# SeanNobel/speech-decoding

Hardware: AMD Instinct MI355X
Metric: train segments/sec (Gwilliams2022 208ch x 360, top-10 retrieval acc alongside) (higher is better)
Workload: dtype bf16; 1 GPU; Gwilliams2022-shaped MEG: 208 ch x 360 samples, 27 subjects, F=1024, batch 256/GPU, fwd+CLIP loss+top-k+bwd+Adam (BASELINE configs[1]); global_batch=256, seq_len=360, parallelism=dp1

## Files before the change

### include/sd_amd.h

```cpp
#ifndef SD_AMD_H
#define SD_AMD_H
#include <stddef.h>
#include <stdint.h>

#ifdef __cplusplus
extern "C" {
#endif

#define SDA_ABI_VERSION 4
#define SDA_ROW_PAD 16
#define SDA_CH_ALIGN 64

enum { SDA_F32 = 0, SDA_BF16 = 1, SDA_F16 = 2 };

enum { SDA_EPI_GELU = 1,
       SDA_EPI_GLU_BWD = 4,
       SDA_EPI_GLU = 2,
       SDA_CONV_SINGLE_TILE = 4096,
       SDA_CONV_PAIR_TILES = 8192,
       SDA_CONV_ONE_PER_CU = 32768,
       SDA_CONV_FLAT_TILES = 16384,
       SDA_CONV_FLAT_STAGGER = 1024,
       SDA_CONV_WIDE_TILES = 524288,
       SDA_CONV_WAVE_PRIO = 1048576,
// ... 95 lines not shown
                                    float* dgamma, float* dbeta, float* coef, void* dx, int B, int T, int Cp, int dtype,
                                    void* stream);
int sda_bn_gelu_backward_apply_dg(const void* dy, const void* x, const float* mean, const float* rstd,
                               const float* gamma, const float* beta, int C, const float* dgamma,
                               const float* dbeta, double count, float* coef , void* dx,
                               int B, int T, int Cp, int dtype, void* stream);

int sda_reduce_scratch_floats(int Cp);

int sda_zero_pad_rows(void* buf, int B, int T, int Cp, int dtype, void* stream);
int sda_fill_zero(void* p, long nbytes, void* stream);
int sda_gather_samples(const void* table, const long* idx, void* dst, int B, long sample_bytes, void* stream);
int sda_gather_windows(const void* table, long table_rows, const int32_t* starts, int M, const long* idx, void* dst, int B, int T,
                       long row_bytes, void* stream);
int sda_scalar_mul(const float* a, const float* b, float* out, int n, void* stream);

int sda_glu_forward(const void* x, void* y, int B, int T, int Ch, int dtype, void* stream);
int sda_glu_backward(const void* x, const void* dy, void* dx, int B, int T, int Ch, int dtype, void* stream);
int sda_gelu_backward(const void* u, const void* dz, void* du, int B, int T, int Cp, int dtype, void* stream);
int sda_reduce_scratch_rows(int B, int T);
int sda_glu_backward_colsum(const void* x, const void* dy, void* dx, float* colsum, float* scratch, int B, int T,
                            int Ch, int dtype, void* stream);
int sda_gelu_backward_colsum(const void* u, const void* dz, void* du, float* colsum, float* scratch, int B, int T,
                             int Cp, int dtype, void* stream);
int sda_glu_backward_colsum_og(const void* out, const void* gate, const void* dy, void* dx, float* colsum, float* scratch,
                               int B, int T, int Ch, int dtype, void* stream);
int sda_colsum(const void* x, float* out, float* scratch , int B, int T,
               int Cp, int dtype, void* stream);

enum { SDA_WGRAD_FLAT_ROWS = 1   };
typedef struct sda_wgrad_args {
  const void* dy;
  const void* x;
  float* g;
  void* out_e;
  const void* sub;
  const float* rscale;
  const float* out_scale;
  const int32_t* perm;
  const int32_t* seg_start;
  int nseg, B, T, Cout_p, Cin_p, KS, dil;
  long dy_pitch, x_pitch, out_pitch;
  long row0, sample_rows;
  long rows_limit;
  long dy_zero_row;
  int co_valid;
  int dtype;
  const float* acc_scale;
  int flags;
} sda_wgrad_args;
int sda_wgrad_gemm(const sda_wgrad_args* a, void* stream);
int sda_wgrad_tile_m(int Cout_p);
int sda_reduce_slabs(const float* src, float* dst, int nslabs, long n, void* stream);
int sda_sim_gemm_ksplit(int M, int N, long K, int dtype);
int sda_sim_gemm(const void* X, const void* W, float* partial, int M, int N, int Np, long K, long pitch, int ksplit, int dtype,
                 void* stream);
int sda_sim_gemm_windows(const void* X, long x_pitch, const void* table, const int32_t* starts, int base_row, long row_elems,
                         float* partial, int M, int N, int Np, long K, int ksplit, int dtype, void* stream);
long sda_sim_gemm_windows_span(long row_elems);
int sda_window_sumsq(const float* row_sq, const int32_t* starts, float* out, int M, int T, void* stream);

int sda_sa_weights_forward(const float* z, const float* cos_t, const float* sin_t, const float* mask,
                           float* W, void* Wp, float* scratch , int D1, int K2,
                           int C, int D1p, int Cp, int dtype, void* stream);
int sda_sa_scratch_floats(int D1, int K2, int C);
int sda_sa_softmax_pack(const float* a, int a_pitch, const float* mask, float* W, void* Wp, int D1, int C, int D1p,
                        int Cp, int dtype, void* stream);
int sda_sa_softmax_backward(const float* dWd, int dwd_pitch, const float* W, const float* mask, float* da,
                            int da_pitch, int D1, int C, void* stream);
int sda_sa_weights_backward(const float* dWd, const float* W, const float* mask, const float* cosT,
                            const float* sinT, float* dz, int D1, int K2, int C, int Cp, void* stream);

int sda_clip_logits_stats(const float* S, long s_pitch, const float* ysq, const float* zsq, const float* temp,
                          float* logits, float* row_max, float* row_sum, float* col_lse, float* diag , float* row_lse ,
                          int Bm, int Bn, int col0, void* stream);
int sda_clip_grad(const float* logits, const float* row_lse, const float* col_lse, const float* ysq,
                  const float* zsq, const float* temp, float inv_norm, int col0, void* G, long g_pitch,
                  float* rscale, float* cscale, float* colpart, float* scalars, int Bm, int Bn, int dtype, void* stream);
int sda_clip_grad_y(const float* logits, const float* row_lse, const float* col_lse, const float* zsq,
                    const float* zsq_all, int nz, int col0, void* Gy, long gy_pitch, int seg, int seg_pitch,
                    float* part, int Bm, int Bn, int dtype, void* stream);
int sda_clip_grad_y_finish(const float* part, int nparts, int Bg, const float* ysq, const float* zsq_all, int nz,
                           const float* temp, float inv_norm, int row0, int nrows, float* rscale_y, float* cscale_y,
                           void* stream);
int sda_clip_dz_supported(int Bm, int Bn, long row_elems, int dtype);
int sda_clip_dz(const void* G, long g_pitch, const void* Y, const void* Z, void* out, const float* cscale, const float* rscale,
                const float* out_scale, int Bm, int Bn, long row_elems, int dtype, void* stream);
int sda_clip_ranks(const float* logits, const float* diag, int32_t* cnt, int Bm, int Bn, int col0, void* stream);
long sda_retrieval_scores_floats(int n, int M, int chunk_cols);
int sda_retrieval_select(const float* S, const float* qsq, const float* csq, const int64_t* labels, int64_t* indices,
                         float* scores, int32_t* ranks, int n, int M, int k, int chunk_cols, void* stream);
int sda_retrieval_class_reduce(const float* S, const float* qsq, const float* csq, const int32_t* order, const int32_t* offsets,
                               float* out, float* row_lse, long out_pitch, int n, int M, int C, int chunk_cols, float scale,
                               int mode, void* stream);
int sda_retrieval_pool_rows(const float* V, long v_pitch, const int32_t* rows, const int32_t* group_offsets, float* out,
                            long out_pitch, int N, int G, int C, void* stream);
int sda_clip_merge_rows(const float* all, int world, int Bg, float* lse, float* diag, void* stream);
int sda_device_count(void);
int sda_stream_create_cumask(const uint32_t* mask, int nwords, void** stream);
int sda_stream_create_priority(int priority, void** stream);
int sda_stream_destroy(void* stream);
int sda_set_cu_limit(int cus);

typedef struct sda_pgemm_args {
  const float* A;
  const float* B;
// ... 95 lines not shown
```

### speech_decoding_amd/blocks.py

```python
from __future__ import annotations

from dataclasses import dataclass, field
from typing import Dict, Optional

import numpy as np
import torch

from . import lib as L
from . import layers
from . import ops

FWD_FLAGS = L.CONV_PAIR_TILES
BWD_FLAGS = L.CONV_WAVE_PRIO


def rows_in(X: torch.Tensor, Cc: int, dtype):
    if X.dtype not in ops.COMPUTE_DTYPES:
        raise L.SdaError(f"input of dtype {X.dtype}: the modules take float32, bfloat16 or float16")
    return ops.rows_of(X, Cc, dtype, ops.new_rows_uninit)


def grad_rows(dY: torch.Tensor, Cc: int, dtype) -> torch.Tensor:
    return ops.rows_of(dY, Cc, dtype, ops.new_rows_uninit)[0]

# ... 49 lines not shown
    dX = ops.input_grad(dY, c.Wp, None, c.B, Cc, c.T, c.x_dtype) if want_x else None
    dz = None
    if want_z:
        dz = layers.sa_z_grad(dY, c.Xt, c.B, c.T, *_segments(c.B, dY, c.Xt), c.W, c.mask, *sa.transposed_tables(), sa.z.shape[1],
                              sa.gemm_tables()[1])
    return dX, dz


def spatial_attention_forward(sa, X: torch.Tensor, mask, need_grad: bool):
    B, Cc, T = X.shape
    Xt, _ = rows_in(X, Cc, sa.compute_dtype)
    y, W, Wp = sa_forward(sa, Xt, B, T, mask, sa.compute_dtype)
    return y, (SACtx(B, T, Xt, W, Wp, mask, X.dtype) if need_grad else None)


@dataclass
class SBCtx:
    sa: SACtx
    h_sa: torch.Tensor
    h_c: torch.Tensor
    widx: torch.Tensor
    subj: Optional[tuple] = None
    params: list = field(default_factory=list)
    versions: list = field(default_factory=list)


def _sb_plans(sb):
    D1p = L.pad_channels(sb.D1)

    def build(f, b):
        layers.add_subject_block_packs(f, b, sb.conv.weight, sb.conv.bias, sb.subject_layer.weight, D1p)
        return f, b
    return _plans(sb, sb.conv.weight.device, build)


def _sb_sources(sb) -> Dict[str, torch.Tensor]:
    return {"sb_w": sb.conv.weight.detach(), "sb_b": sb.conv.bias.detach(), "subj_w": sb.subject_layer.weight.detach()}


def subject_block_forward(sb, X: torch.Tensor, sidx: np.ndarray, mask, need_grad: bool, want_subj_grad: bool):
    B, Cc, T = X.shape
    dt, dev, D1, S = sb.compute_dtype, X.device, sb.D1, sb.num_subjects
    D1p = L.pad_channels(D1)
    widx = ops.UPLOADER.upload("blocks.widx", sidx.astype(np.int32), dev)
    Xt, _ = rows_in(X, Cc, dt)
    h_sa, W, Wp = sa_forward(sb.spatial_attention, Xt, B, T, mask, dt)
    pk = _sb_plans(sb)[0].run(_sb_sources(sb))
    h_c = ops.conv_gemm(h_sa, pk["sb_w"], _new(B, T, D1p, dt, dev), B=B, T=T, KS=1, dil=0, bias=pk["sb_b"], alg_dims=(D1, D1))
    y = ops.conv_gemm(h_c, pk["subj_w"], _new(B, T, D1p, dt, dev), B=B, T=T, KS=1, dil=0, widx=widx, alg_dims=(D1, D1))
    if not need_grad:
        return y, None
    c = SBCtx(SACtx(B, T, Xt, W, Wp, mask, X.dtype), h_sa, h_c, widx)
    if want_subj_grad:
        plan = layers.subject_plan(sidx, S, *layers.subject_tiles_blocks(D1p))
        c.subj = (ops.UPLOADER.upload("blocks.subj_perm", plan.perm, dev), ops.UPLOADER.upload("blocks.subj_seg", plan.seg_start, dev),
                  plan.r)
    return y, c


def subject_block_backward(sb, c: SBCtx, dY: torch.Tensor, want: Dict[str, bool]) -> Dict[str, torch.Tensor]:
    _check_versions(c)
    B, T, dt, dev = c.sa.B, c.sa.T, sb.compute_dtype, dY.device
    D1, S = sb.D1, sb.num_subjects
    D1p = L.pad_channels(D1)
    g: Dict[str, torch.Tensor] = {}
    if want["subj_w"]:
        g["subj_w"] = layers.subject_wgrad(dY, c.h_c, B, T, *c.subj, S, D1)
    if not (want["sb_w"] or want["sb_b"] or want["z"] or want["X"]):
        return g
    pkT = _sb_plans(sb)[1].run(_sb_sources(sb))
    dh_c = ops.conv_gemm(dY, pkT["subj_w"], _new(B, T, D1p, dt, dev), B=B, T=T, KS=1, dil=0, widx=c.widx, alg_dims=(D1, D1),
                         flags=BWD_FLAGS)
    if want["sb_w"]:
        g["sb_w"] = _wgrad(dh_c, c.h_sa, B, T, 1, 0, D1, D1)
    if want["sb_b"]:
        g["sb_b"] = ops.colsum(dh_c, B, T, ops.reduce_scratch(D1p, dev))[:D1]
    if want["z"] or want["X"]:
        dh_sa = ops.conv_gemm(dh_c, pkT["sb_w"], _new(B, T, D1p, dt, dev), B=B, T=T, KS=1, dil=0, alg_dims=(D1, D1),
                              flags=BWD_FLAGS)
        g["X"], g["z"] = sa_backward(sb.spatial_attention, c.sa, dh_sa, want["X"], want["z"])
    return g


CB_PARAMS = ("c0w", "c0b", "bn0w", "bn0b", "c1w", "c1b", "bn1w", "bn1b", "c2w", "c2b")


def cb_params(cb):
    return [cb.conv0.weight, cb.conv0.bias, cb.batchnorm0.weight, cb.batchnorm0.bias, cb.conv1.weight, cb.conv1.bias,
            cb.batchnorm1.weight, cb.batchnorm1.bias, cb.conv2.weight, cb.conv2.bias]


@dataclass
class CBCtx:
    B: int
    T: int
    x: torch.Tensor
    x_rows: bool
    x_dtype: torch.dtype
    h: list
    a: list
    bn: list
    c2: torch.Tensor
    params: list = field(default_factory=list)
    versions: list = field(default_factory=list)


def _cb_plans(cb):
    def build(f, b):
        layers.add_conv_block_packs(f, b, "", [(c.weight, c.bias) for c in (cb.conv0, cb.conv1, cb.conv2)], cb.D2,
                                    L.pad_channels(cb.in_channels))
        return f, b
    return _plans(cb, cb.conv0.weight.device, build)


def _cb_sources(cb) -> Dict[str, torch.Tensor]:
    return {n: p.detach() for n, p in zip(CB_PARAMS, cb_params(cb)) if not n.startswith("bn")}


def conv_block_forward(cb, X: torch.Tensor, need_grad: bool):
    B, Cc, T = X.shape
# ... 81 lines not shown
```

### speech_decoding_amd/csrc/param_ops.hip

```cpp
#include <math.h>

#include "sd_common.h"

namespace sda {

__device__ inline int glu_unmap(int cop, int Cout, int half, int half_p, int tile = 0) {
  if (half == 0) return cop < Cout ? cop : -1;
  if (tile > 0) {
    const int j = cop / (2 * tile), w = cop - j * 2 * tile;
    const int r = j * tile + (w < tile ? w : w - tile);
    if (w < tile) return r < half ? r : -1;
    return r < Cout - half ? half + r : -1;
  }
  if (cop < half_p) return cop < half ? cop : -1;
  const int r = cop - half_p;
  return r < Cout - half ? half + r : -1;
}
__device__ inline int glu_map(int co, int half, int half_p) { return (half == 0 || co < half) ? co : half_p + co - half; }

__device__ inline float packed_weight_value(const float* __restrict__ w, size_t i, int Cout, int Cin, int KS, int Cout_p,
                                            int Cin_p, int mode, int half, int half_p, int tile) {
  int co, ci, tap;
  size_t q = i;
  if (mode == 0) {
// ... 49 lines not shown

__device__ inline void slab_add(float& s, float v) { s += v; }
__device__ inline void slab_add(float4& s, const float4& v) { s.x += v.x; s.y += v.y; s.z += v.z; s.w += v.w; }

template <typename V>
__device__ inline V ordered_slab_sum(const float* __restrict__ slabs, int nslabs, size_t slab, size_t src) {
  V sum = {};
  int k = 0;
  for (; k + 8 <= nslabs; k += 8) {
    V v[8];
#pragma unroll
    for (int j = 0; j < 8; ++j) v[j] = *reinterpret_cast<const V*>(slabs + (size_t)(k + j) * slab + src);
#pragma unroll
    for (int j = 0; j < 8; ++j) slab_add(sum, v[j]);
  }
  for (; k < nslabs; ++k) slab_add(sum, *reinterpret_cast<const V*>(slabs + (size_t)k * slab + src));
  return sum;
}

__global__ void reduce_unpack_wgrad_kernel(const float* __restrict__ slabs, int nslabs, float* __restrict__ dst, int Cout,
                                           int Cin, int KS, int Cout_p, int Cin_p, int half, int half_p) {
  const size_t total = (size_t)Cout * Cin * KS;
  const size_t slab = (size_t)KS * Cout_p * Cin_p;
  for (size_t i = (size_t)blockIdx.x * blockDim.x + threadIdx.x; i < total; i += (size_t)gridDim.x * blockDim.x) {
    size_t q = i;
    const int ci = q % Cin; q /= Cin;
    const int co = q % Cout; q /= Cout;
    const int tap = (int)q;
    const size_t src = ((size_t)tap * Cout_p + glu_map(co, half, half_p)) * Cin_p + ci;
    dst[((size_t)co * Cin + ci) * KS + tap] = ordered_slab_sum<float>(slabs, nslabs, slab, src);
  }
}

__global__ __launch_bounds__(256) void reduce_unpack_wgrad_vec_kernel(const float* __restrict__ slabs, int nslabs, float* __restrict__ dst,
                                                                      int Cout, int Cin, int KS, int Cout_p, int Cin_p, int half, int half_p) {
  const int cin4 = Cin >> 2;
  const size_t total = (size_t)Cout * cin4 * KS;
  const size_t slab = (size_t)KS * Cout_p * Cin_p;
  for (size_t i = (size_t)blockIdx.x * blockDim.x + threadIdx.x; i < total; i += (size_t)gridDim.x * blockDim.x) {
    size_t q = i;
    const int c4 = q % cin4; q /= cin4;
    const int co = q % Cout; q /= Cout;
    const int tap = (int)q;
    const size_t src = ((size_t)tap * Cout_p + glu_map(co, half, half_p)) * Cin_p + 4 * c4;
    const float4 sum = ordered_slab_sum<float4>(slabs, nslabs, slab, src);
    float* o = dst + ((size_t)co * Cin + 4 * c4) * KS + tap;
    o[0] = sum.x; o[KS] = sum.y; o[2 * KS] = sum.z; o[3 * KS] = sum.w;
  }
}

__global__ void reduce_slabs_kernel(const float* __restrict__ src, float* __restrict__ dst, int nslabs, long n) {
  for (long i = (long)blockIdx.x * blockDim.x + threadIdx.x; i < n; i += (long)gridDim.x * blockDim.x)
    dst[i] = ordered_slab_sum<float>(src, nslabs, (size_t)n, (size_t)i);
}

__global__ void pack_vector_kernel(const float* __restrict__ v, float* __restrict__ dst, int C, int Cp, int half, int half_p) {
  const int i = blockIdx.x * blockDim.x + threadIdx.x;
  if (i >= Cp) return;
  const int c = glu_unmap(i, C, half, half_p);
  dst[i] = c >= 0 ? v[c] : 0.f;
}
__global__ void unpack_vector_kernel(const float* __restrict__ g, float* __restrict__ dst, int C, int half, int half_p) {
  const int i = blockIdx.x * blockDim.x + threadIdx.x;
  if (i < C) dst[i] = g[glu_map(i, half, half_p)];
}

static inline int ew_grid(size_t total) {
  size_t g = (total + 255) / 256;
  return (int)(g < 1 ? 1 : (g > 4096 ? 4096 : g));
}

}

using namespace sda;

extern "C" int sda_pack_conv_weight(const float* w, void* dst, int nW, int Cout, int Cin, int KS, int Cout_p,
                                    int Cin_p, int mode, int glu_half, int glu_half_p, int dtype, void* stream) {
  if (!w || !dst || nW < 1 || Cout > Cout_p || Cin > Cin_p || (mode != 0 && mode != 1)) { set_error("pack_conv_weight: bad arguments"); return -1; }
  if (glu_half && (glu_half_p < glu_half || glu_half_p + (Cout - glu_half) > Cout_p)) { set_error("pack_conv_weight: bad GLU split"); return -1; }
  hipStream_t st = (hipStream_t)stream;
  const size_t total = (size_t)nW * KS * Cout_p * Cin_p;
  SDA_DISPATCH(dtype, hipLaunchKernelGGL(pack_conv_weight_kernel<E>, dim3(ew_grid(total)), dim3(256), 0, st, w,
                                         (E*)dst, nW, Cout, Cin, KS, Cout_p, Cin_p, mode, glu_half, glu_half_p));
  return check_launch("pack_conv_weight");
}

extern "C" int sda_unpack_conv_wgrad(const float* g, float* dst, int nW, int Cout, int Cin, int KS, int Cout_p,
                                     int Cin_p, int glu_half, int glu_half_p, void* stream) {
  if (!g || !dst) { set_error("unpack_conv_wgrad: null"); return -1; }
  const size_t total = (size_t)nW * Cout * Cin * KS;
  hipLaunchKernelGGL(unpack_conv_wgrad_kernel, dim3(ew_grid(total)), dim3(256), 0, (hipStream_t)stream, g, dst, nW,
                     Cout, Cin, KS, Cout_p, Cin_p, glu_half, glu_half_p);
  return check_launch("unpack_conv_wgrad");
}

template <bool COEF>
__device__ __forceinline__ void adam_multi_body(const sda_adam_desc& d, float lr, float beta1, float beta2, float eps, float bc1,
                                                float bc2_sqrt, float coef) {
  const float step_size = lr / bc1;
  for (long i = ((long)blockIdx.x * 256 + threadIdx.x) * 4; i < d.n; i += (long)gridDim.x * 1024) {
    if (i + 4 <= d.n && d.aligned) {
      float4 p = *reinterpret_cast<float4*>(d.param + i);
      float4 g = *reinterpret_cast<const float4*>(d.grad + i);
      if (COEF) { g.x = __fmul_rn(g.x, coef); g.y = __fmul_rn(g.y, coef); g.z = __fmul_rn(g.z, coef); g.w = __fmul_rn(g.w, coef); }
      float4 m = *reinterpret_cast<float4*>(d.exp_avg + i), v = *reinterpret_cast<float4*>(d.exp_avg_sq + i);
#define SDA_ADAM(f)                                                     \
// ... 33 lines not shown
}

extern "C" int sda_adam_multi(const sda_adam_desc* descs_dev, int n, long max_n, float lr, float beta1, float beta2, float eps,
                              long step, void* stream) {
  if (!descs_dev || n < 1 || max_n < 1 || step < 1) { set_error("adam_multi: bad arguments"); return -1; }
  const double bc1 = 1.0 - pow((double)beta1, (double)step);
  const double bc2 = 1.0 - pow((double)beta2, (double)step);
  long gx = (max_n + 1023) / 1024;
  if (gx > 256) gx = 256;
  hipLaunchKernelGGL(adam_multi_kernel, dim3((unsigned)gx, (unsigned)n), dim3(256), 0, (hipStream_t)stream, descs_dev, lr, beta1,
                     beta2, eps, (float)bc1, (float)sqrt(bc2));
  return check_launch("adam_multi");
}

extern "C" int sda_adam_multi_guarded(const sda_adam_desc* descs_dev, int n, long max_n, float lr, float beta1, float beta2,
                                      float eps, const double* state, void* stream) {
  if (!descs_dev || !state || n < 1 || max_n < 1) { set_error("adam_multi_guarded: bad arguments (null pointer, n or max_n < 1)"); return -1; }
  long gx = (max_n + 1023) / 1024;
  if (gx > 256) gx = 256;
  hipLaunchKernelGGL(adam_multi_guarded_kernel, dim3((unsigned)gx, (unsigned)n), dim3(256), 0, (hipStream_t)stream, descs_dev, lr,
                     beta1, beta2, eps, state);
  return check_launch("adam_multi_guarded");
}

extern "C" int sda_pack_multi(const sda_pack_desc* descs_dev, int n, long max_total, int dtype, void* stream) {
  if (!descs_dev || n < 1 || max_total < 1) { set_error("pack_multi: bad arguments"); return -1; }
  hipStream_t st = (hipStream_t)stream;
  long gx = (max_total + 1023) / 1024;
  if (gx > 512) gx = 512;
  SDA_DISPATCH(dtype, hipLaunchKernelGGL(pack_multi_kernel<E>, dim3((unsigned)gx, (unsigned)n), dim3(256), 0, st, descs_dev));
  return check_launch("pack_multi");
}

extern "C" int sda_reduce_unpack_wgrad(const float* slabs, int nslabs, float* dst, int Cout, int Cin, int KS, int Cout_p,
                                       int Cin_p, int glu_half, int glu_half_p, void* stream) {
  if (!slabs || !dst || nslabs < 1) { set_error("reduce_unpack_wgrad: bad arguments"); return -1; }
  const size_t total = (size_t)Cout * Cin * KS;
  if (Cin % 4 == 0 && Cin_p % 4 == 0 && (reinterpret_cast<uintptr_t>(slabs) & 15) == 0) {
    hipLaunchKernelGGL(reduce_unpack_wgrad_vec_kernel, dim3(ew_grid(total / 4)), dim3(256), 0, (hipStream_t)stream, slabs, nslabs, dst,
                       Cout, Cin, KS, Cout_p, Cin_p, glu_half, glu_half_p);
    return check_launch("reduce_unpack_wgrad");
  }
  hipLaunchKernelGGL(reduce_unpack_wgrad_kernel, dim3(ew_grid(total)), dim3(256), 0, (hipStream_t)stream, slabs, nslabs, dst,
                     Cout, Cin, KS, Cout_p, Cin_p, glu_half, glu_half_p);
  return check_launch("reduce_unpack_wgrad");
}

extern "C" int sda_reduce_slabs(const float* src, float* dst, int nslabs, long n, void* stream) {
  if (!src || !dst || nslabs < 1 || n < 1) { set_error("reduce_slabs: bad arguments"); return -1; }
  hipLaunchKernelGGL(reduce_slabs_kernel, dim3(ew_grid((size_t)n)), dim3(256), 0, (hipStream_t)stream, src, dst, nslabs, n);
  return check_launch("reduce_slabs");
}

extern "C" int sda_pack_vector(const float* v, float* dst, int C, int Cp, int glu_half, int glu_half_p, void* stream) {
  if (!v || !dst || C > Cp) { set_error("pack_vector: bad arguments"); return -1; }
  hipLaunchKernelGGL(pack_vector_kernel, dim3((Cp + 255) / 256), dim3(256), 0, (hipStream_t)stream, v, dst, C, Cp,
                     glu_half, glu_half_p);
  return check_launch("pack_vector");
}

extern "C" int sda_unpack_vector(const float* g, float* dst, int C, int Cp, int glu_half, int glu_half_p, void* stream) {
  if (!g || !dst || C > Cp) { set_error("unpack_vector: bad arguments"); return -1; }
  hipLaunchKernelGGL(unpack_vector_kernel, dim3((C + 255) / 256), dim3(256), 0, (hipStream_t)stream, g, dst, C,
                     glu_half, glu_half_p);
  return check_launch("unpack_vector");
}
```

### speech_decoding_amd/engine.py

```python
from __future__ import annotations

from dataclasses import dataclass, field
from typing import Dict, List, Optional

import ast
import os

import numpy as np
import torch

from . import lib as L
from . import layers
from . import ops
from .clip import ClipBlockStats, ClipCtx, clip_backward, clip_backward_y, clip_block_finish, clip_block_stats, clip_forward


@dataclass
class EncoderDims:
    C: int
    S: int
    D1: int
    D2: int
    F: int
    K: int

    @property
    def Cp(self): return L.pad_channels(self.C)
    @property
    def D1p(self): return L.pad_channels(self.D1)
    @property
    def D2p(self): return L.pad_channels(self.D2)
    @property
    def F1(self): return 2 * self.D2
    @property
    def F1p(self): return L.pad_channels(2 * self.D2)
    @property
    def Fp(self): return L.pad_channels(self.F)


@dataclass
class EncoderCtx:
    B: int
    T: int
    gen: int
    training: bool
    bufs: Dict[str, torch.Tensor] = field(default_factory=dict)
    packed: Dict[str, torch.Tensor] = field(default_factory=dict)
    bn: Dict[str, tuple] = field(default_factory=dict)
    mask: Optional[torch.Tensor] = None
    widx: Optional[torch.Tensor] = None
    subj_perm: Optional[torch.Tensor] = None
    subj_seg: Optional[torch.Tensor] = None
    subj_slices: int = 1
    W_sa: Optional[torch.Tensor] = None
    packed_T: Dict[str, torch.Tensor] = field(default_factory=dict)
    packed_T_ready: Optional[torch.cuda.Event] = None
    glu_fused: bool = False
    composed: Optional[tuple] = None
    param_grads: bool = True
    x_dtype: Optional[torch.dtype] = None
    W_x: Optional[torch.Tensor] = None


@dataclass
class _Forward:
    eng: "EncoderEngine"
    P: Dict[str, torch.Tensor]
    ctx: EncoderCtx
    dev: torch.device
    main: torch.cuda.Stream
    need_grad: bool
    need_dx: bool
    eps: float
    momentum: float
    k3_flags: int
    count: float
    packed_ready: Optional[torch.cuda.Event] = None
    flip: Dict[int, int] = field(default_factory=dict)

    def rows(self, name, Cp):
        B, T = self.ctx.B, self.ctx.T
        if not self.need_grad:
            name = f"pp{self.flip.setdefault(Cp, 0) % 3}"
            self.flip[Cp] += 1
        return self.eng._rows(name, B, T, Cp, self.dev, "train" if self.need_grad else "eval")


class _Backward:
    __slots__ = ("eng", "P", "ctx", "B", "T", "dev", "pg", "main", "side", "grads", "pending", "scratch", "overlap", "world")

    def __init__(self, eng: "EncoderEngine", P, ctx: EncoderCtx, dev, main):
        d = eng.d
        self.eng, self.P, self.ctx, self.B, self.T, self.dev, self.main = eng, P, ctx, ctx.B, ctx.T, dev, main
        self.grads: Dict[str, torch.Tensor] = {}
        self.pg = ctx.param_grads
        self.scratch = ops.reduce_scratch(max(d.Fp, 2 * d.D2p, d.F1p), dev)
        self.pending = []
        self.overlap = eng.group is not None and eng.overlap_grad_allreduce
        self.side = eng._side_stream(dev) if eng.wgrad_side_stream else None
        self.world = eng.world

    def flush(self, names):
        if not self.overlap or not self.pg:
            return
        import torch.distributed as dist
        from .distributed import side_group
# ... 184 lines not shown
            layers.add_conv_block_packs(f, b, f"b{k}.", [(P[f"b{k}.c{j}w"], P[f"b{k}.c{j}b"]) for j in range(3)], d.D2,
                                        d.D1p if k == 0 else d.D2p, glu_tile)
        f.add_weight("f1w", P["f1w"], d.F1p, d.D2p)
        f.add_vector("f1b", P["f1b"], d.F1p)
        f.add_weight("f2w", P["f2w"], d.Fp, d.F1p)
        f.add_vector("f2b", P["f2b"], d.Fp)
        b.add_weight("f1w", P["f1w"], d.F1p, d.D2p, mode=1)
        b.add_weight("f2w", P["f2w"], d.Fp, d.F1p, mode=1)
        self._fwd_plan, self._bwd_plan, self._plan_key = f, b, key
        return f, b

    def forward(self, P: Dict[str, torch.Tensor], X: torch.Tensor, subject_idxs, *, training: bool,
                mask: Optional[torch.Tensor], need_grad: bool, momentum: float = 0.1, eps: float = 1e-5,
                need_dx: bool = False, param_grads: bool = True) -> EncoderCtx:
        B, Cc, T = X.shape
        assert Cc == self.d.C, f"expected {self.d.C} channels, got {Cc}"
        dev = X.device
        if need_grad:
            self._gen += 1
        self._touch_shape("train" if need_grad else "eval", B, T)
        ctx = EncoderCtx(B=B, T=T, gen=self._gen, training=training)
        ctx.glu_fused = self.glu_fused
        if need_dx and not need_grad:
            raise L.SdaError("EncoderEngine.forward: need_dx needs need_grad")
        ctx.param_grads = bool(param_grads or not need_dx)
        ctx.x_dtype = X.dtype if need_dx else None
        ctx.mask = mask
        k3_flags = L.CONV_PAIR_TILES
        if self.flat_forward:
            k3_flags |= L.CONV_FLAT_TILES | L.CONV_FLAT_STAGGER
        f = _Forward(self, P, ctx, dev, torch.cuda.current_stream(dev), need_grad, need_dx, eps, momentum, k3_flags,
                     count=float(B) * T * self.world)

        self._fwd_subjects(f, subject_idxs)
        Xt = ctx.bufs["Xt"] = self._fwd_pack(f, X)
        x = self._fwd_subject_block(f, Xt)
        for k in range(5):
            x = self._fwd_conv_block(f, k, x)
        Zt = self._fwd_projections(f, x)
        if not need_grad:
            ctx.bufs = {"Z": Zt}
            ctx.packed = {}
        return ctx

    def _fwd_subjects(self, f: _Forward, subject_idxs):
        d, ctx = self.d, f.ctx
        B = ctx.B
        sidx = layers.subject_indices(subject_idxs, B, d.S)
        up = ops.UPLOADER.upload
        ctx.widx = up(("widx", "train" if f.need_grad else "eval"), sidx.astype(np.int32), f.dev)
        if not (f.need_grad and ctx.param_grads):
            return
        tiles = layers.subject_tiles_composed(d.D2p, d.Cp) if self.composed else layers.subject_tiles_three_conv(d.D1p)
        plan = layers.subject_plan(sidx, d.S, *tiles)
        ctx.subj_perm = up("subj_perm", plan.perm, f.dev)
        ctx.subj_seg = up("subj_seg", plan.seg_start, f.dev)
        ctx.subj_slices = plan.r

    def _fwd_pack(self, f: _Forward, X):
        d, ctx, P = self.d, f.ctx, f.P
        fwd_plan, bwd_plan = self._plans(P, f.dev)
        side = self._side_stream(f.dev) if self.pack_on_side_stream else None
        Xt = f.rows("Xt", d.Cp)
        if side is not None:
            ev = torch.cuda.Event()
            ev.record(f.main)
            side.wait_event(ev)
        with torch.cuda.stream(side):
            ctx.packed.update(fwd_plan.run(P))
            ops.pack_rows(X, Xt, ones_channel=d.C if self.composed else None)
            if side is not None:
                X.record_stream(side)
                f.packed_ready = torch.cuda.Event()
                f.packed_ready.record(side)
            if f.need_grad:
                ctx.packed_T = bwd_plan.run(P)
                if side is not None:
                    ctx.packed_T_ready = torch.cuda.Event()
                    ctx.packed_T_ready.record(side)
        return Xt

    def _fwd_subject_block(self, f: _Forward, Xt):
        d, ctx, P, dev = self.d, f.ctx, f.P, f.dev
        B, T, pk = ctx.B, ctx.T, ctx.packed
        composed = self.composed
        ctx.W_sa, Wp = ops.sa_weights_forward(P["z"], P["cos"], P["sin"], ctx.mask, d.D1p, d.Cp,
                                              torch.float32 if composed else self.dtype, fwd_table=P.get("sa_tab_f"))
        if not composed:
            ctx.W_x = Wp if f.need_dx else None
            if f.packed_ready is not None:
                self._wait("packed operands (forward)", f.main, f.packed_ready)
            h_sa = ops.conv_gemm(Xt, Wp, f.rows("h_sa", d.D1p), B=B, T=T, KS=1, dil=0, alg_dims=(d.C, d.D1))
            h_c = ops.conv_gemm(h_sa, pk["sb_w"], f.rows("h_c", d.D1p), B=B, T=T, KS=1, dil=0, bias=pk["sb_b"],
                                alg_dims=(d.D1, d.D1))
            x = ops.conv_gemm(h_c, pk["subj_w"], f.rows("x0", d.D1p), B=B, T=T, KS=1, dil=0, widx=ctx.widx, alg_dims=(d.D1, d.D1))
            ctx.bufs.update(h_sa=h_sa, h_c=h_c, x0=x)
            return x
        Wd = Wp[0, 0, : d.D1, : d.C]
        Ws = P["subj_w"][..., 0]
        T1aug = torch.empty((d.D1, d.C + 1), dtype=torch.float32, device=dev)
        ops.param_gemm(P["sb_w"][..., 0], Wd, out=T1aug[:, : d.C])
        ops.copy3d(T1aug[:, d.C:], P["sb_b"][:, None])
        key = ("wtot", str(dev), self.dtype)
        Wtot = self._const.get(key)
        if f.need_dx:
            Wtot = ctx.W_x = ops.zeros((d.S, 1, d.D1p, d.Cp), self.dtype, dev)
        elif Wtot is None:
            Wtot = self._const[key] = torch.zeros((d.S, 1, d.D1p, d.Cp), dtype=self.dtype, device=dev)
        ops.param_gemm(Ws, T1aug, out=Wtot[:, 0, : d.D1, : d.C + 1])
        if f.need_grad:
# ... 151 lines not shown
        dc2 = b.tmp(f"dc2.{k}", 2 * d.D2p)
        if not pg:
            if ctx.glu_fused:
                ops.glu_backward_og(bufs[f"x{k + 1}"], bufs[f"b{k}.g"], dx, dc2, B, T)
            else:
                ops.glu_backward(bufs[f"b{k}.c2"], dx, dc2, B, T)
        elif ctx.glu_fused:
            grads[f"b{k}.c2b"] = ops.bias_grad(ops.glu_backward_colsum_og(bufs[f"x{k + 1}"], bufs[f"b{k}.g"], dx, dc2, B, T, scratch),
                                               2 * d.D2, **glu)
        else:
            grads[f"b{k}.c2b"] = ops.bias_grad(ops.glu_backward_colsum(bufs[f"b{k}.c2"], dx, dc2, B, T, scratch), 2 * d.D2, **glu)
        da1, tstats = b.dgrad(dc2, f"b{k}.c2w", b.tmp("da", d.D2p), 3, dil[2], bn=(bufs[f"b{k}.h1"], ctx.bn[f"b{k}.bn1"][2]))
        grads[f"b{k}.c2w"] = b.wgrad(dc2, bufs[f"b{k}.a1"], 3, dil[2], 2 * d.D2, d.D2, **glu)
        for j in (1, 0):
            bnp = f"b{k}.bn{j}"
            mean, rstd, _ = ctx.bn[bnp]
            dh = b.tmp(f"dh.{k}.{j}", d.D2p)
            sync = self.group is not None and ctx.training
            dgam, dbet = ops.bn_gelu_backward(da1, bufs[f"b{k}.h{j}"], mean, rstd, P[bnp + "w"], P[bnp + "b"], dh, B, T,
                                              scratch, count=float(B) * T * world if ctx.training else float("inf"),
                                              allreduce=self._allreduce if sync else None, tile_stats=tstats)
            if sync and pg:
                both = dgam._base if dgam._base is not None else torch.stack([dgam, dbet])
                if b.side is not None:
                    both.record_stream(b.side)
                scaled = b.on_side(lambda: both / world)
                dgam, dbet = scaled[0], scaled[1]
            if pg:
                grads[bnp + "w"], grads[bnp + "b"] = dgam[: d.D2], dbet[: d.D2]
                grads[f"b{k}.c{j}b"] = null_bias[2 * k + j] if ctx.training else ops.bias_grad(ops.colsum(dh, B, T, scratch), d.D2)
            src, ci, ci_p = (bufs[f"b{k}.a0"], d.D2, d.D2p) if j == 1 else (bufs[f"x{k}"], cin, cin_p)
            key = f"b{k}.c{j}w"
            res = dh if (j == 1 or k > 0) else None
            out = b.tmp("da", d.D2p) if j == 1 else b.tmp("dxB" if k % 2 == 0 else "dxA", ci_p)
            if k == 0 and j == 0 and ctx.composed is not None and ctx.x_dtype is None:
                da1 = None
            else:
                da1, tstats = b.dgrad(dh, key, out, 3, dil[j], res=res,
                                      bn=(bufs[f"b{k}.h0"], ctx.bn[f"b{k}.bn0"][2]) if j == 1 else None)
            grads[key] = b.wgrad(dh, src, 3, dil[j], d.D2, ci)
        b.flush([f"b{k}.c2w", f"b{k}.c2b", f"b{k}.c1w", f"b{k}.c1b", f"b{k}.bn1w", f"b{k}.bn1b",
                 f"b{k}.c0w", f"b{k}.c0b", f"b{k}.bn0w", f"b{k}.bn0b"])
        return da1, dh

    def _bwd_subject_composed(self, b: _Backward, dx, dh0, w0cat):
        d, ctx, P, grads = self.d, b.ctx, b.P, b.grads
        B, T, dev = b.B, b.T, b.dev
        if ctx.x_dtype is not None:
            grads["X"] = ops.input_grad(dx, ctx.W_x, ctx.widx, B, d.C, T, ctx.x_dtype)
        if not b.pg:
            return
        Wd, T1aug, Ws = ctx.composed
        W0cat, w0cat_ready = w0cat
        r = ctx.subj_slices
        M = ops.wgrad_gemm(dh0, ctx.bufs["Xt"], B=B, T=T, KS=3, dil=layers.block_dilations(0)[0], perm=ctx.subj_perm,
                           seg_start=ctx.subj_seg, nseg=r * d.S, flat_rows=True)
        if r > 1:
            M = ops.reduce_slabs(M.view(r, -1))
        if w0cat_ready is not None:
            self._wait("W0cat copy (side stream)", b.main, w0cat_ready)
        G = ops.param_gemm(W0cat.view(d.D1, 3 * d.D2p), M.view(d.S, 3 * d.D2p, d.Cp)[:, :, : d.C + 1])
        grads["subj_w"] = b.on_side(lambda: ops.param_gemm(G, T1aug.t()).view(d.S, d.D1, d.D1, 1))
        part = ops.param_gemm(Ws.transpose(1, 2), G)
        dT1f = ops.reduce_slabs(part.view(d.S, -1)).view(d.D1, d.C + 1)
        dT1 = dT1f[:, : d.C]
        grads["sb_b"], grads["sb_w"] = b.on_side(lambda: (
            ops.copy3d(torch.empty(d.D1, dtype=torch.float32, device=dev), dT1f[:, d.C]),
            ops.param_gemm(dT1, Wd.t()).unsqueeze(-1)))
        dWd = ops.param_gemm(P["sb_w"][..., 0].t(), dT1)
        grads["z"] = ops.sa_weights_backward(dWd, ctx.W_sa, ctx.mask, P["cosT"], P["sinT"], P["z"].shape[1],
                                             bwd_table=P.get("sa_tab_b"))

    def _bwd_subject_three_conv(self, b: _Backward, dhs):
        d, ctx, P, grads, pg = self.d, b.ctx, b.P, b.grads, b.pg
        B, T, bufs = b.B, b.T, ctx.bufs
        if pg:
            grads["subj_w"] = b.on_side(lambda: layers.subject_wgrad(dhs, bufs["h_c"], B, T, ctx.subj_perm, ctx.subj_seg,
                                                                     ctx.subj_slices, d.S, d.D1))
        dh_c, _ = b.dgrad(dhs, "subj_w", b.tmp("dh_c", d.D1p), 1, 0, widx=ctx.widx)
        if pg:
            grads["sb_w"] = b.wgrad(dh_c, bufs["h_sa"], 1, 0, d.D1, d.D1)
            grads["sb_b"] = ops.bias_grad(ops.colsum(dh_c, B, T, b.scratch), d.D1)
        dh_sa, _ = b.dgrad(dh_c, "sb_w", b.tmp("dh_sa", d.D1p), 1, 0)
        if ctx.x_dtype is not None:
            grads["X"] = ops.input_grad(dh_sa, ctx.W_x, None, B, d.C, T, ctx.x_dtype)
        if not pg:
            return
        nseg = layers.uniform_nseg(B, d.D1p, d.Cp)
        _, seg = self._uniform_segments(B, nseg, b.dev)
        grads["z"] = layers.sa_z_grad(dh_sa, bufs["Xt"], B, T, seg, nseg, ctx.W_sa, ctx.mask, P["cosT"], P["sinT"], P["z"].shape[1],
                                      P.get("sa_tab_b"))
```

### speech_decoding_amd/layers.py

```python
from __future__ import annotations

from typing import NamedTuple

import numpy as np
import torch

from . import lib as L
from . import ops


def block_dilations(k: int):
    return 2 ** ((2 * k) % 5), 2 ** ((2 * k + 1) % 5), 2


def subject_indices(subject_idxs, B: int, S: int) -> np.ndarray:
    sidx = torch.as_tensor(subject_idxs).detach().to("cpu").to(torch.int64).numpy()
    if sidx.shape != (B,):
        raise ValueError("subject_idxs must have shape (B,)")
    if (sidx < 0).any() or (sidx >= S).any():
        raise IndexError("subject index out of range")
    return sidx


WGRAD_TARGET_WGS = 256


def wgrad_ntiles(Cout_p: int, Cin_p: int, tile_n: int = 64) -> int:
    return (Cout_p // ops.wgrad_tile_m(Cout_p)) * (Cin_p // tile_n)


def uniform_segment_count(B: int, ntiles: int) -> int:
    nseg = 8 * max(1, round(WGRAD_TARGET_WGS / (8 * max(1, ntiles))))
    return int(min(B, nseg)) if B >= 8 else int(max(1, min(B, nseg)))


def uniform_segment_edges(B: int, nseg: int) -> np.ndarray:
    return np.floor(np.linspace(0, B, nseg + 1)).astype(np.int32)


def subject_slices(B: int, present: int, ntiles: int) -> int:
    return int(max(1, min(max(1, B // present), round(WGRAD_TARGET_WGS / max(1, ntiles * present)))))


def subject_segments(sidx: np.ndarray, S: int, r: int):
    order = np.argsort(sidx, kind="stable").astype(np.int32)
    bounds = np.searchsorted(sidx[order], np.arange(S + 1)).astype(np.int64)
    lo, hi = bounds[:-1], bounds[1:]
    cuts = [lo + ((hi - lo) * j) // r for j in range(r + 1)]
    seg = np.empty(r * S + 1, dtype=np.int32)
    parts, pos = [], 0
    for j in range(r):
        for s in range(S):
            a_, b_ = int(cuts[j][s]), int(cuts[j + 1][s])
            seg[j * S + s] = pos
            parts.append(order[a_:b_])
            pos += b_ - a_
    seg[r * S] = pos
    perm = np.concatenate(parts).astype(np.int32) if parts else order
    return perm, seg


def uniform_nseg(B: int, Cout_p: int, Cin_p: int, tile_n: int = 64) -> int:
    return uniform_segment_count(B, wgrad_ntiles(Cout_p, Cin_p, tile_n))


def subject_tiles_composed(D2p, Cp): return D2p, Cp, 64
def subject_tiles_three_conv(D1p): return D1p, D1p, 128 if D1p % 128 == 0 else 64
def subject_tiles_blocks(D1p): return D1p, D1p, 64


class SubjectPlan(NamedTuple):
    perm: np.ndarray
    seg_start: np.ndarray
    r: int


def subject_plan(sidx: np.ndarray, S: int, Cout_p: int, Cin_p: int, tile_n: int) -> SubjectPlan:
    r = subject_slices(sidx.shape[0], max(1, int(np.unique(sidx).size)), wgrad_ntiles(Cout_p, Cin_p, tile_n))
    return SubjectPlan(*subject_segments(sidx, S, r), r)


def conv_wgrad(dy, x, B, T, KS, dil, Cout, Cin, seg, nseg, glu_half=0, glu_half_p=0) -> torch.Tensor:
    slabs = ops.wgrad_gemm(dy, x, B=B, T=T, KS=KS, dil=dil, seg_start=seg, nseg=nseg, alg_dims=(Cin, Cout), flat_rows=True)
    return ops.reduce_unpack_wgrad(slabs, Cout, Cin, KS, glu_half=glu_half, glu_half_p=glu_half_p)


def subject_wgrad(dy, h_c, B, T, perm, seg, r, S, D1) -> torch.Tensor:
    D1p = dy.shape[1]
    slabs = ops.wgrad_gemm(dy, h_c, B=B, T=T, KS=1, dil=0, perm=perm, seg_start=seg, nseg=r * S, flat_rows=True)
    if r > 1:
        slabs = ops.reduce_slabs(slabs.view(r, -1)).view(S, 1, D1p, D1p)
    return ops.unpack_conv_wgrad(slabs, S, D1, D1, 1, D1p, D1p)


def sa_z_grad(dy, Xt, B, T, seg, nseg, W, mask, cosT, sinT, K, bwd_table) -> torch.Tensor:
    dWd = ops.reduce_slabs(ops.wgrad_gemm(dy, Xt, B=B, T=T, KS=1, dil=0, seg_start=seg, nseg=nseg))
    return ops.sa_weights_backward(dWd, W, mask, cosT, sinT, K, bwd_table=bwd_table)


def add_conv_block_packs(f, b, prefix: str, convs, D2: int, cin_p: int, glu_tile: int = 0):
    D2p = L.pad_channels(D2)
    glu = dict(glu_half=D2, glu_half_p=D2p)
    for j in (0, 1):
        w, bias = convs[j]
        ci_p = cin_p if j == 0 else D2p
        f.add_weight(f"{prefix}c{j}w", w, D2p, ci_p)
        f.add_vector(f"{prefix}c{j}b", bias, D2p)
        b.add_weight(f"{prefix}c{j}w", w, D2p, ci_p, mode=1)
    w, bias = convs[2]
    f.add_weight(prefix + "c2w", w, 2 * D2p, D2p, glu_tile=glu_tile, **glu)
    f.add_vector(prefix + "c2b", bias, 2 * D2p, glu_tile=glu_tile, **glu)
    b.add_weight(prefix + "c2w", w, 2 * D2p, D2p, mode=1, **glu)


def add_subject_block_packs(f, b, sb_w, sb_b, subj_w, D1p: int):
    f.add_weight("sb_w", sb_w, D1p, D1p)
    f.add_vector("sb_b", sb_b, D1p)
    f.add_weight("subj_w", subj_w, D1p, D1p)
    b.add_weight("sb_w", sb_w, D1p, D1p, mode=1)
    b.add_weight("subj_w", subj_w, D1p, D1p, mode=1)
```

### speech_decoding_amd/ops.py

```python
from __future__ import annotations

import ctypes as C
from typing import Optional

import numpy as np
import torch

from . import lib as L

_DT = {torch.float32: L.F32, torch.bfloat16: L.BF16, torch.float16: L.F16}
COMPUTE_DTYPES = tuple(_DT)


def dt_code(dtype: torch.dtype) -> int:
    try:
        return _DT[dtype]
    except KeyError:
        raise L.SdaError(f"unsupported compute dtype {dtype}; use torch.float32, torch.bfloat16 or torch.float16")


def _p(t: Optional[torch.Tensor]):
    return None if t is None else t.data_ptr()


# ... 693 lines not shown
    return cs


def colsum(x, B, T, scratch):
    out = torch.empty(x.shape[1], dtype=torch.float32, device=x.device)
    L.check(L.load().sda_colsum(_p(x), _p(out), _p(scratch), B, T, x.shape[1], dt_code(x.dtype), _st()), "colsum")
    return out


def wgrad_tile_m(Cout_p: int) -> int:
    return L.load().sda_wgrad_tile_m(Cout_p)


def splitk_tile_co(Np: int) -> int:
    return 160 if Np % 160 == 0 else (128 if Np % 128 == 0 else 64)


def bias_grad(cs, C, glu_half=0, glu_half_p=0):
    if glu_half == 0 or glu_half_p == glu_half:
        return cs[:C]
    return unpack_vector(cs, C, glu_half, glu_half_p)


def wgrad_args(dy, x, *, B, T, Cout_p, Cin_p, KS, dil, dy_pitch, x_pitch, rows_limit, dtype, flags=0, g=None, perm=None,
               seg_start=None, nseg=1, row0=L.ROW_PAD, sample_rows=None, dy_zero_row=0, out_e=None, out_pitch=0, co_valid=0,
               sub=None, rscale=None, acc_scale=None, out_scale=None) -> L.WgradArgs:
    return L.WgradArgs(dy, x, g, out_e, sub, rscale, out_scale, perm, seg_start, nseg, B, T, Cout_p, Cin_p, KS, dil, dy_pitch, x_pitch,
                       out_pitch, row0, L.rows_tp(T) if sample_rows is None else sample_rows, rows_limit, dy_zero_row, co_valid, dtype,
                       acc_scale, flags)


def wgrad_gemm(dy, x, *, B, T, KS, dil, perm=None, seg_start=None, nseg=1, alg_dims=None, flat_rows=False):
    g = torch.empty((nseg, KS, dy.shape[1], x.shape[1]), dtype=torch.float32, device=x.device)
    if nseg > 1 and seg_start is None:
        raise L.SdaError("wgrad_gemm: nseg > 1 needs seg_start")
    a = wgrad_args(_p(dy), _p(x), B=B, T=T, Cout_p=dy.shape[1], Cin_p=x.shape[1], KS=KS, dil=dil, dy_pitch=dy.shape[1],
                   x_pitch=x.shape[1], rows_limit=x.shape[0], dtype=dt_code(x.dtype), g=_p(g), perm=_p(perm), seg_start=_p(seg_start),
                   nseg=nseg, flags=L.WGRAD_FLAT_ROWS if flat_rows else 0)
    cin, cout = alg_dims if alg_dims is not None else (x.shape[1], dy.shape[1])
    _launch("wgrad_gemm", lambda: (("wgrad_gemm", str(x.dtype).replace("torch.", ""), wgrad_tile_m(dy.shape[1]), KS),
                                   2.0 * B * T * KS * cin * cout), L.load().sda_wgrad_gemm, a, "wgrad_gemm")
    return g


def reduce_slabs(slabs: torch.Tensor) -> torch.Tensor:
    n = slabs[0].numel()
    if slabs.shape[0] == 1:
        return slabs[0]
    out = torch.empty_like(slabs[0])
    L.check(L.load().sda_reduce_slabs(_p(slabs), _p(out), slabs.shape[0], n, _st()), "reduce_slabs")
    return out


def matmul_tn_typed(G, Ym, out, sub, rscale, *, M_rows, N_valid, K_cols, pitch, out_scale=None, acc_scale=None):
    if G.shape[0] < M_rows + 1:
        raise L.SdaError("matmul_tn_typed: G needs one trailing all-zero row")
    a = wgrad_args(_p(G), _p(Ym), B=1, T=M_rows, Cout_p=G.shape[1], Cin_p=K_cols, KS=1, dil=0, dy_pitch=G.stride(0), x_pitch=pitch,
                   rows_limit=M_rows, dtype=dt_code(Ym.dtype), row0=0, sample_rows=0, dy_zero_row=M_rows, out_e=_p(out),
                   out_pitch=pitch, co_valid=N_valid, sub=_p(sub), rscale=_p(rscale), acc_scale=_p(acc_scale), out_scale=_p(out_scale))
    L.check(L.load().sda_wgrad_gemm(C.byref(a), _st()), "wgrad_gemm(typed)")
    return out


def clip_dz(G, Yt, Zt, out, rscale, cscale, *, Bm, Bn, row_elems, out_scale=None):
    if G.stride(1) != 1:
        raise L.SdaError("clip_dz: the coefficient matrix needs unit column stride")
    if L.load().sda_clip_dz_supported(Bm, Bn, row_elems, dt_code(Yt.dtype)):
        L.check(L.load().sda_clip_dz(_p(G), G.stride(0), _p(Yt), _p(Zt), _p(out), _p(cscale), _p(rscale), _p(out_scale), Bm, Bn, row_elems,
                                     dt_code(Yt.dtype), _st()), "clip_dz")
        return out
    return matmul_tn_typed(G, Yt, out, Zt, rscale, M_rows=Bm, N_valid=Bn, K_cols=row_elems, pitch=row_elems, out_scale=out_scale,
                           acc_scale=cscale)


def sa_gemm_tables(cos_t: torch.Tensor, sin_t: torch.Tensor):
    K2, Cc = cos_t.shape
    both = torch.stack([cos_t, sin_t], dim=-1)
    fwd = both.permute(1, 0, 2).reshape(Cc, 2 * K2).contiguous()
    Cq = (Cc + 63) // 64 * 64
    bwd = torch.zeros((2 * K2, Cq), dtype=torch.float32, device=cos_t.device)
    bwd[:, :Cc] = both.permute(0, 2, 1).reshape(2 * K2, Cc)
    return fwd, bwd


def sa_weights_forward(z, cos_t, sin_t, mask, D1p, Cp, dtype, fwd_table=None):
    D1, K2 = z.shape
    Cc = cos_t.shape[1]
    zr = torch.view_as_real(z).contiguous().view(D1, 2 * K2)
    W = torch.empty((D1, Cc), dtype=torch.float32, device=z.device)
    Wp = torch.empty((1, 1, D1p, Cp), dtype=dtype, device=z.device)
    if fwd_table is not None and (2 * K2) % 64 == 0:
        a = matmul_nt_splitk(zr, fwd_table, D1, Cc, 2 * K2, 2 * K2)
        L.check(L.load().sda_sa_softmax_pack(_p(a), a.shape[1], _p(mask), _p(W), _p(Wp), D1, Cc, D1p, Cp, dt_code(dtype), _st()),
                "sa_softmax_pack")
        return W, Wp
    scratch = torch.empty(L.load().sda_sa_scratch_floats(D1, K2, Cc), dtype=torch.float32, device=z.device)
    L.check(L.load().sda_sa_weights_forward(_p(zr), _p(cos_t), _p(sin_t), _p(mask), _p(W), _p(Wp), _p(scratch), D1, K2, Cc, D1p, Cp,
                                            dt_code(dtype), _st()), "sa_weights_forward")
    return W, Wp


def sa_weights_backward(dWd, W, mask, cosT, sinT, K2, bwd_table=None):
    D1, Cc = W.shape
    if bwd_table is not None and (2 * K2) % 64 == 0:
        bwd = bwd_table
        Cq = bwd.shape[1]
# ... 344 lines not shown
```

Before: 37140 segments/s.

## Balance per-subject wgrad segments by row cap and reduce variable-size slab groups

Measured after the change: 37100 segments/s. No clear change (-0.1%).

```diff
diff --git a/include/sd_amd.h b/include/sd_amd.h
--- a/include/sd_amd.h
+++ b/include/sd_amd.h
@@ -171,6 +171,7 @@
 int sda_wgrad_gemm(const sda_wgrad_args* a, void* stream);
 int sda_wgrad_tile_m(int Cout_p);
 int sda_reduce_slabs(const float* src, float* dst, int nslabs, long n, void* stream);
+int sda_reduce_slab_groups(const float* src, float* dst, const int* group_start, int ngroups, long n, void* stream);
 int sda_sim_gemm_ksplit(int M, int N, long K, int dtype);
 int sda_sim_gemm(const void* X, const void* W, float* partial, int M, int N, int Np, long K, long pitch, int ksplit, int dtype,
                  void* stream);
diff --git a/speech_decoding_amd/blocks.py b/speech_decoding_amd/blocks.py
--- a/speech_decoding_amd/blocks.py
+++ b/speech_decoding_amd/blocks.py
@@ -125,9 +125,7 @@
         return y, None
     c = SBCtx(SACtx(B, T, Xt, W, Wp, mask, X.dtype), h_sa, h_c, widx)
     if want_subj_grad:
-        plan = layers.subject_plan(sidx, S, *layers.subject_tiles_blocks(D1p))
-        c.subj = (ops.UPLOADER.upload("blocks.subj_perm", plan.perm, dev), ops.UPLOADER.upload("blocks.subj_seg", plan.seg_start, dev),
-                  plan.r)
+        c.subj = layers.upload_subject_plan(layers.subject_plan(sidx, S, *layers.subject_tiles_blocks(D1p)), "blocks.subj", dev)
     return y, c
 
 
@@ -138,7 +136,7 @@
     D1p = L.pad_channels(D1)
     g: Dict[str, torch.Tensor] = {}
     if want["subj_w"]:
-        g["subj_w"] = layers.subject_wgrad(dY, c.h_c, B, T, *c.subj, S, D1)
+        g["subj_w"] = layers.subject_wgrad(dY, c.h_c, B, T, c.subj, S, D1)
     if not (want["sb_w"] or want["sb_b"] or want["z"] or want["X"]):
         return g
     pkT = _sb_plans(sb)[1].run(_sb_sources(sb))
diff --git a/speech_decoding_amd/csrc/param_ops.hip b/speech_decoding_amd/csrc/param_ops.hip
--- a/speech_decoding_amd/csrc/param_ops.hip
+++ b/speech_decoding_amd/csrc/param_ops.hip
@@ -125,6 +125,18 @@
 __global__ void reduce_slabs_kernel(const float* __restrict__ src, float* __restrict__ dst, int nslabs, long n) {
   for (long i = (long)blockIdx.x * blockDim.x + threadIdx.x; i < n; i += (long)gridDim.x * blockDim.x)
     dst[i] = ordered_slab_sum<float>(src, nslabs, (size_t)n, (size_t)i);
+}
+
+template <typename V>
+__global__ __launch_bounds__(256) void reduce_slab_groups_kernel(const float* __restrict__ src, float* __restrict__ dst,
+                                                                 const int* __restrict__ group_start, long n) {
+  constexpr int W = (int)(sizeof(V) / sizeof(float));
+  const int g = blockIdx.y;
+  const int s0 = group_start[g], ns = group_start[g + 1] - s0;
+  const float* __restrict__ base = src + (size_t)s0 * n;
+  float* __restrict__ out = dst + (size_t)g * n;
+  for (long i = ((long)blockIdx.x * blockDim.x + threadIdx.x) * W; i < n; i += (long)gridDim.x * blockDim.x * W)
+    *reinterpret_cast<V*>(out + i) = ordered_slab_sum<V>(base, ns, (size_t)n, (size_t)i);
 }
 
 __global__ void pack_vector_kernel(const float* __restrict__ v, float* __restrict__ dst, int C, int Cp, int half, int half_p) {
@@ -264,6 +276,17 @@
   return check_launch("reduce_slabs");
 }
 
+extern "C" int sda_reduce_slab_groups(const float* src, float* dst, const int* group_start, int ngroups, long n, void* stream) {
+  if (!src || !dst || !group_start || ngroups < 1 || ngroups > 65535 || n < 1) { set_error("reduce_slab_groups: bad arguments"); return -1; }
+  const bool vec = n % 4 == 0 && ((reinterpret_cast<uintptr_t>(src) | reinterpret_cast<uintptr_t>(dst)) & 15) == 0;
+  size_t gx = ((size_t)(vec ? n / 4 : n) + 255) / 256;
+  if (gx > 1024) gx = 1024;
+  const dim3 grid((unsigned)gx, (unsigned)ngroups);
+  if (vec) hipLaunchKernelGGL(reduce_slab_groups_kernel<float4>, grid, dim3(256), 0, (hipStream_t)stream, src, dst, group_start, n);
+  else hipLaunchKernelGGL(reduce_slab_groups_kernel<float>, grid, dim3(256), 0, (hipStream_t)stream, src, dst, group_start, n);
+  return check_launch("reduce_slab_groups");
+}
+
 extern "C" int sda_pack_vector(const float* v, float* dst, int C, int Cp, int glu_half, int glu_half_p, void* stream) {
   if (!v || !dst || C > Cp) { set_error("pack_vector: bad arguments"); return -1; }
   hipLaunchKernelGGL(pack_vector_kernel, dim3((Cp + 255) / 256), dim3(256), 0, (hipStream_t)stream, v, dst, C, Cp,
diff --git a/speech_decoding_amd/engine.py b/speech_decoding_amd/engine.py
--- a/speech_decoding_amd/engine.py
+++ b/speech_decoding_amd/engine.py
@@ -49,9 +49,7 @@
     bn: Dict[str, tuple] = field(default_factory=dict)
     mask: Optional[torch.Tensor] = None
     widx: Optional[torch.Tensor] = None
-    subj_perm: Optional[torch.Tensor] = None
-    subj_seg: Optional[torch.Tensor] = None
-    subj_slices: int = 1
+    subj: Optional[layers.SubjectSegments] = None
     W_sa: Optional[torch.Tensor] = None
     packed_T: Dict[str, torch.Tensor] = field(default_factory=dict)
     packed_T_ready: Optional[torch.cuda.Event] = None
@@ -342,10 +340,7 @@
         if not (f.need_grad and ctx.param_grads):
             return
         tiles = layers.subject_tiles_composed(d.D2p, d.Cp) if self.composed else layers.subject_tiles_three_conv(d.D1p)
-        plan = layers.subject_plan(sidx, d.S, *tiles)
-        ctx.subj_perm = up("subj_perm", plan.perm, f.dev)
-        ctx.subj_seg = up("subj_seg", plan.seg_start, f.dev)
-        ctx.subj_slices = plan.r
+        ctx.subj = layers.upload_subject_plan(layers.subject_plan(sidx, d.S, *tiles), "subj", f.dev)
 
     def _fwd_pack(self, f: _Forward, X):
         d, ctx, P = self.d, f.ctx, f.P
@@ -603,11 +598,10 @@
             return
         Wd, T1aug, Ws = ctx.composed
         W0cat, w0cat_ready = w0cat
-        r = ctx.subj_slices
-        M = ops.wgrad_gemm(dh0, ctx.bufs["Xt"], B=B, T=T, KS=3, dil=layers.block_dilations(0)[0], perm=ctx.subj_perm,
-                           seg_start=ctx.subj_seg, nseg=r * d.S, flat_rows=True)
-        if r > 1:
-            M = ops.reduce_slabs(M.view(r, -1))
+        M = ops.wgrad_gemm(dh0, ctx.bufs["Xt"], B=B, T=T, KS=3, dil=layers.block_dilations(0)[0], perm=ctx.subj.perm,
+                           seg_start=ctx.subj.seg, nseg=ctx.subj.nseg, flat_rows=True)
+        if not ctx.subj.one_each:
+            M = ops.reduce_slab_groups(M, ctx.subj.groups, d.S)
         if w0cat_ready is not None:
             self._wait("W0cat copy (side stream)", b.main, w0cat_ready)
         G = ops.param_gemm(W0cat.view(d.D1, 3 * d.D2p), M.view(d.S, 3 * d.D2p, d.Cp)[:, :, : d.C + 1])
@@ -626,8 +620,7 @@
         d, ctx, P, grads, pg = self.d, b.ctx, b.P, b.grads, b.pg
         B, T, bufs = b.B, b.T, ctx.bufs
         if pg:
-            grads["subj_w"] = b.on_side(lambda: layers.subject_wgrad(dhs, bufs["h_c"], B, T, ctx.subj_perm, ctx.subj_seg,
-                                                                     ctx.subj_slices, d.S, d.D1))
+            grads["subj_w"] = b.on_side(lambda: layers.subject_wgrad(dhs, bufs["h_c"], B, T, ctx.subj, d.S, d.D1))
         dh_c, _ = b.dgrad(dhs, "subj_w", b.tmp("dh_c", d.D1p), 1, 0, widx=ctx.widx)
         if pg:
             grads["sb_w"] = b.wgrad(dh_c, bufs["h_sa"], 1, 0, d.D1, d.D1)
diff --git a/speech_decoding_amd/layers.py b/speech_decoding_amd/layers.py
--- a/speech_decoding_amd/layers.py
+++ b/speech_decoding_amd/layers.py
@@ -69,15 +69,62 @@
 def subject_tiles_blocks(D1p): return D1p, D1p, 64
 
 
+SUBJECT_TARGET_WGS = WGRAD_TARGET_WGS
+
+
+def subject_cap(counts: np.ndarray, ntiles: int, target_wgs: int = None) -> int:
+    counts = np.asarray(counts, dtype=np.int64)
+    counts = counts[counts > 0]
+    if counts.size == 0:
+        return 1
+    want = max(int(counts.size), int(round((SUBJECT_TARGET_WGS if target_wgs is None else target_wgs) / max(1, ntiles))))
+    for cap in range(1, int(counts.max()) + 1):
+        if int((-(-counts // cap)).sum()) <= want:
+            return cap
+    return int(counts.max())
+
+
+def balanced_subject_segments(sidx: np.ndarray, S: int, cap: int):
+    order = np.argsort(sidx, kind="stable").astype(np.int32)
+    bounds = np.searchsorted(sidx[order], np.arange(S + 1)).astype(np.int64)
+    seg, group = [0], np.zeros(S + 1, dtype=np.int32)
+    for s in range(S):
+        lo, n = int(bounds[s]), int(bounds[s + 1] - bounds[s])
+        k = -(-n // cap)
+        seg.extend(lo + (n * j) // k for j in range(1, k + 1))
+        group[s + 1] = group[s] + k
+    return order, np.asarray(seg, dtype=np.int32), group
+
+
 class SubjectPlan(NamedTuple):
     perm: np.ndarray
     seg_start: np.ndarray
-    r: int
+    group_start: np.ndarray
+    cap: int
+
+    @property
+    def nseg(self) -> int:
+        return int(self.seg_start.shape[0]) - 1
 
 
-def subject_plan(sidx: np.ndarray, S: int, Cout_p: int, Cin_p: int, tile_n: int) -> SubjectPlan:
-    r = subject_slices(sidx.shape[0], max(1, int(np.unique(sidx).size)), wgrad_ntiles(Cout_p, Cin_p, tile_n))
-    return SubjectPlan(*subject_segments(sidx, S, r), r)
+def subject_plan(sidx: np.ndarray, S: int, Cout_p: int, Cin_p: int, tile_n: int, target_wgs: int = None) -> SubjectPlan:
+    cap = subject_cap(np.bincount(sidx, minlength=S), wgrad_ntiles(Cout_p, Cin_p, tile_n), target_wgs)
+    return SubjectPlan(*balanced_subject_segments(sidx, S, cap), cap)
+
+
+class SubjectSegments(NamedTuple):
+    perm: torch.Tensor
+    seg: torch.Tensor
+    groups: torch.Tensor
+    nseg: int
+    one_each: bool
+
+
+def upload_subject_plan(plan: SubjectPlan, key: str, dev) -> SubjectSegments:
+    up = ops.UPLOADER.upload
+    return SubjectSegments(up(key + ".perm", plan.perm, dev), up(key + ".seg", plan.seg_start, dev),
+                           up(key + ".groups", plan.group_start, dev), plan.nseg,
+                           bool(np.array_equal(plan.group_start, np.arange(plan.group_start.shape[0]))))
 
 
 def conv_wgrad(dy, x, B, T, KS, dil, Cout, Cin, seg, nseg, glu_half=0, glu_half_p=0) -> torch.Tensor:
@@ -85,11 +132,11 @@
     return ops.reduce_unpack_wgrad(slabs, Cout, Cin, KS, glu_half=glu_half, glu_half_p=glu_half_p)
 
 
-def subject_wgrad(dy, h_c, B, T, perm, seg, r, S, D1) -> torch.Tensor:
+def subject_wgrad(dy, h_c, B, T, subj: SubjectSegments, S, D1) -> torch.Tensor:
     D1p = dy.shape[1]
-    slabs = ops.wgrad_gemm(dy, h_c, B=B, T=T, KS=1, dil=0, perm=perm, seg_start=seg, nseg=r * S, flat_rows=True)
-    if r > 1:
-        slabs = ops.reduce_slabs(slabs.view(r, -1)).view(S, 1, D1p, D1p)
+    slabs = ops.wgrad_gemm(dy, h_c, B=B, T=T, KS=1, dil=0, perm=subj.perm, seg_start=subj.seg, nseg=subj.nseg, flat_rows=True)
+    if not subj.one_each:
+        slabs = ops.reduce_slab_groups(slabs, subj.groups, S)
     return ops.unpack_conv_wgrad(slabs, S, D1, D1, 1, D1p, D1p)
 
 
diff --git a/speech_decoding_amd/ops.py b/speech_decoding_amd/ops.py
--- a/speech_decoding_amd/ops.py
+++ b/speech_decoding_amd/ops.py
@@ -769,6 +769,15 @@
     return out
 
 
+def reduce_slab_groups(slabs: torch.Tensor, group_start: torch.Tensor, ngroups: int) -> torch.Tensor:
+    if group_start.dtype != torch.int32 or group_start.numel() != ngroups + 1 or not group_start.is_cuda:
+        raise L.SdaError("reduce_slab_groups: group_start must be a device int32 tensor of ngroups + 1 entries")
+    n = slabs[0].numel()
+    out = torch.empty((ngroups,) + tuple(slabs.shape[1:]), dtype=torch.float32, device=slabs.device)
+    L.check(L.load().sda_reduce_slab_groups(_p(slabs), _p(out), _p(group_start), ngroups, n, _st()), "reduce_slab_groups")
+    return out
+
+
 def matmul_tn_typed(G, Ym, out, sub, rscale, *, M_rows, N_valid, K_cols, pitch, out_scale=None, acc_scale=None):
     if G.shape[0] < M_rows + 1:
         raise L.SdaError("matmul_tn_typed: G needs one trailing all-zero row")
```
